# sxyu/avatar

Measured on AMD Instinct MI355X. Metric: Gauss-Newton iterations/sec (30k-pt cloud, 10 shape + 24-joint pose), higher is better.
Workload: dtype f64

## Files before the change

### avatar_amd/api.py

```python
from __future__ import annotations

import ctypes as C
import math
import os

import numpy as np

from . import capi
from .capi import AvtError, ModelArrays, Options, Profile, Stats, bptr, check, dptr, iptr


def rot_to_quat(R):
    m = np.asarray(R, np.float64).reshape(-1, 3, 3)
    N = m.shape[0]
    q = np.empty((N, 4))
    tr = m[:, 0, 0] + m[:, 1, 1] + m[:, 2, 2]
    pos = tr > 0
    with np.errstate(invalid="ignore", divide="ignore"):
        t = np.sqrt(np.where(pos, tr, 0.0) + 1.0)
        ti = 0.5 / t
        qa = np.stack([(m[:, 2, 1] - m[:, 1, 2]) * ti, (m[:, 0, 2] - m[:, 2, 0]) * ti, (m[:, 1, 0] - m[:, 0, 1]) * ti, 0.5 * t], 1)
        i = np.where(m[:, 1, 1] > m[:, 0, 0], 1, 0)
        ar = np.arange(N)
        i = np.where(m[:, 2, 2] > m[ar, i, i], 2, i)
# ... 437 lines not shown

    def normal_equations(self, frame=0):
        P = self.model.arrays.P
        H = np.empty((P, P)); g = np.empty(P); cost = C.c_double()
        check(self._lib.avt_get_normal_equations(self.h, C.c_int(frame), dptr(H), dptr(g), C.byref(cost)))
        return H, g, cost.value

    def cost_trace(self, frame=0, n=11):
        buf = np.zeros(64)
        check(self._lib.avt_debug_trace(self.h, C.c_int(frame), dptr(buf)))
        return buf[:n].copy()

    def mfma_count(self, frame=0):
        a, b, c = C.c_longlong(), C.c_longlong(), C.c_longlong()
        check(self._lib.avt_debug_mfma_count(self.h, C.c_int(frame), C.byref(a), C.byref(b), C.byref(c)))
        return {k: (None if v.value < 0 else int(v.value)) for k, v in (("eval_rows", a), ("moments", b), ("solve", c))}

    def nn_sums(self, frame=0):
        V = self.model.numPoints()
        cnt = np.empty(V, np.int32); fsum = np.empty((3, V), np.int64); centre = np.empty(3)
        check(self._lib.avt_debug_nn_sums(self.h, C.c_int(frame), iptr(cnt), fsum.ctypes.data_as(C.POINTER(C.c_longlong)), dptr(centre)))
        return cnt, fsum, centre

    DATA_TERM_ROWS, DATA_TERM_MOMENTS, DATA_TERM_AUTO = 0, 1, 2

    def tuning(self):
        t = capi.Tuning()
        check(self._lib.avt_ctx_get_tuning(self.h, C.byref(t)))
        return t

    def set_tuning(self, **kw):
        t = self.tuning()
        for k, v in kw.items():
            if k not in dict(t._fields_):
                raise KeyError(k)
            setattr(t, k, int(v))
        check(self._lib.avt_ctx_set_tuning(self.h, C.byref(t)))
        return self

    def set_data_term(self, form):
        check(self._lib.avt_set_data_term(self.h, C.c_int(int(form))))

    def data_term(self):
        return int(self._lib.avt_get_data_term(self.h))

    def launch_shape(self):
# ... 175 lines not shown
```

### avatar_amd/capi.py

```python
from __future__ import annotations

import ctypes as C
import os

import numpy as np
import scipy.sparse as sp

_HERE = os.path.dirname(os.path.abspath(__file__))
LIB_PATH = os.environ.get("AVT_LIB", os.path.join(_HERE, "csrc", "libavatar_hip.so"))

c_double_p = C.POINTER(C.c_double)
c_int_p = C.POINTER(C.c_int)
c_ubyte_p = C.POINTER(C.c_ubyte)

AVT_K_NAMES = ["lbs", "visibility", "bucket", "nn", "aggregate", "prepare", "eval", "reduce", "solve", "decide", "moments"]
AVT_K_COUNT = len(AVT_K_NAMES)


class ModelDesc(C.Structure):
    _fields_ = [
        ("num_points", C.c_int), ("num_joints", C.c_int), ("num_shape_keys", C.c_int), ("num_faces", C.c_int),
        ("base_cloud", c_double_p), ("key_clouds", c_double_p), ("parent", c_int_p), ("mesh", c_int_p),
        ("weights_colptr", c_int_p), ("weights_row", c_int_p), ("weights_val", c_double_p),
        ("jreg_colptr", c_int_p), ("jreg_row", c_int_p), ("jreg_val", c_double_p),
# ... 185 lines not shown
    "avt_state_upload_frames": [_vp, C.c_int, c_int_p, c_double_p, c_double_p, c_double_p],
    "avt_state_reset": [_vp],
    "avt_state_download": [_vp, c_double_p, c_double_p, c_double_p, C.POINTER(Stats)],
    "avt_get_correspondences": [_vp, C.c_int, c_int_p],
    "avt_get_cloud": [_vp, C.c_int, c_double_p],
    "avt_get_posed": [_vp, C.c_int, c_double_p, c_double_p, c_double_p],
    "avt_get_normal_equations": [_vp, C.c_int, c_double_p, c_double_p, c_double_p],
    "avt_ctx_get_tuning": [_vp, C.POINTER(Tuning)],
    "avt_ctx_set_tuning": [_vp, C.POINTER(Tuning)],
    "avt_set_data_term": [_vp, C.c_int],
    "avt_get_data_term": [_vp],
    "avt_set_occlusion_render": [_vp, C.c_int, C.c_int, C.c_float, C.c_float, C.c_float, C.c_float],
    "avt_get_visibility": [_vp, C.c_int, c_ubyte_p],
    "avt_set_corr_gate": [_vp, C.c_int, c_double_p],
    "avt_get_corr_gate": [_vp, c_double_p],
    "avt_get_gated": [_vp, C.c_int, c_int_p],
    "avt_set_corr_trim": [_vp, C.c_int, c_double_p, c_double_p, c_double_p, C.c_int],
    "avt_get_corr_trim": [_vp, c_double_p, c_double_p, c_double_p, c_int_p],
    "avt_get_trimmed": [_vp, C.c_int, c_int_p, c_int_p],
    "avt_get_trim_thresholds": [_vp, C.c_int, c_double_p],
    "avt_debug_trace": [_vp, C.c_int, c_double_p],
    "avt_debug_mfma_count": [_vp, C.c_int, C.POINTER(C.c_longlong), C.POINTER(C.c_longlong), C.POINTER(C.c_longlong)],
    "avt_debug_nn_sums": [_vp, C.c_int, c_int_p, C.POINTER(C.c_longlong), c_double_p],
    "avt_launch_shape": [_vp, c_int_p, c_int_p, c_int_p],
    "avt_profile_begin": [_vp],
    "avt_profile_select": [_vp, C.c_uint],
    "avt_profile_end": [_vp, C.POINTER(Profile)],
    "avt_shard_owner": [C.c_int, C.c_int],
    "avt_shard_local_count": [C.c_int, C.c_int, C.c_int],
    "avt_shard_local_index": [C.c_int, C.c_int],
    "avt_shard_global_frame": [C.c_int, C.c_int, C.c_int],
    "avt_model_pack_size": [C.POINTER(ModelDesc), C.POINTER(C.c_size_t)],
    "avt_model_pack": [C.POINTER(ModelDesc), _vp, C.c_size_t],
    "avt_model_unpack": [_vp, C.c_size_t, C.POINTER(_vp)],
    "avt_shard_unique_id": [C.c_char_p],
    "avt_shard_create": [C.c_int, C.c_int, C.c_int, C.c_char_p, C.POINTER(_vp)],
    "avt_shard_create_loopback": [C.c_int, C.c_int, C.c_int, C.c_char_p, C.POINTER(_vp)],
    "avt_shard_create_shm": [C.c_int, C.c_int, C.c_int, C.c_char_p, C.POINTER(_vp)],
    "avt_shard_destroy": [_vp],
    "avt_shard_rank": [_vp],
    "avt_shard_world": [_vp],
    "avt_shard_backend": [_vp],
    "avt_shard_broadcast_model": [_vp, C.c_int, C.POINTER(ModelDesc), C.POINTER(_vp)],
    "avt_shard_scatter_frames": [_vp, _vp, C.c_int, C.c_int, c_double_p, c_int_p, c_int_p, c_double_p, c_double_p, c_double_p],
    "avt_shard_gather_enqueue": [_vp, _vp, C.c_int],
    "avt_shard_gather_wait": [_vp],
# ... 39 lines not shown
```

### avatar_amd/csrc/avt_capi.cpp

```cpp
#include <algorithm>
#include <cmath>
#include <cstdio>
#include <cstdlib>
#include <cstring>
#include <limits>

#include <memory>
#include <mutex>

#include "avt_internal.h"

static std::mutex g_graph_mutex;

int avt_solve_set_attributes();
int avt_eval_set_attributes();
int avt_render_enqueue(avt_ctx* c, int nframes, const int* d_vertex_part, unsigned long long* d_zkey, unsigned char* d_label, int* d_block,
                       double fx, double fy, double cx, double cy, int width, int height);
int avt_paint_enqueue(avt_ctx* c, int nframes, const int* d_vertex_part, unsigned long long* d_dkey, unsigned long long* d_mkey, float* d_fkey,
                      int* d_frank, unsigned char* d_fedge, float* d_depth, unsigned char* d_label, int* d_block, double fx, double fy, double cx,
                      double cy, int width, int height);
void avt_eval_report_occupancy(const AvtDims& d);

namespace {

template <class T>
int dev_alloc(avt_ctx* c, T** p, size_t n) {
    DevBuf<char> b;
    if (b.reserve(std::max<size_t>(n, 1) * sizeof(T))) return 1;
    *p = (T*)b.p;
    c->owned.push_back(std::move(b));
    return 0;
}
template <class T>
int dev_upload(avt_ctx* c, T** p, const std::vector<T>& v) {
    if (dev_alloc(c, p, v.size())) return 1;
    if (!v.empty()) {
        AVT_HIP(hipMemcpyAsync(*p, v.data(), v.size() * sizeof(T), hipMemcpyHostToDevice, c->stream));
        AVT_HIP(hipStreamSynchronize(c->stream));
    }
    return 0;
}

int choose_groups(int nframes, const avt_tuning& tun) {
    int n = nframes >= 44 ? 2 : 1;
    if (tun.groups > 0) n = tun.groups;
    return std::max(1, std::min(std::min(n, AVT_MAX_GROUPS), nframes));
}

int choose_G(int nframes, int ngroups, const avt_tuning& tun);
int plan_groups(avt_ctx* c, int nf) {
    int ngroups = choose_groups(nf, c->tun);
    if ((nf == 2 || nf == 3) && c->tun.groups <= 0) {
        const int g_keep = c->fb.G;
        c->fb.G = choose_G(1, 1, c->tun);
        if (avt_solve_rides(c, 1)) ngroups = nf;
        c->fb.G = g_keep;
    }
    return ngroups;
}

int choose_G(int nframes, int ngroups, const avt_tuning& tun) {
    const int target = nframes >= 128 ? 1536 : (ngroups >= 2 ? (nframes <= 40 ? 512 : 640) : 768);
    const int gcap = std::max(2, std::min(AVT_G_MAX, tun.gcap));
    int g = std::max(2, std::min(gcap, target / std::max(1, nframes)));
    if (nframes >= 7) g = std::min(g, 63);
    if (tun.g > 0) return std::max(1, std::min(g, tun.g));
    return g;
}

extern "C" char** environ;
avt_tuning tuning_from_environment() {
    avt_tuning t;
    std::memset(&t, 0, sizeof t);
    t.use_graph = 1; t.groups = 0; t.g = 0; t.gcap = 128; t.vis_frame_min = 32; t.ride = 1; t.ride_strips = 0; t.ride_sizing_groups = 0;
    t.asm_parts = 1; t.spec_cost = 1; t.xcd_frames = 1; t.literal_dims = 1; t.nspec = AVT_MAX_SPEC; t.nn_force_part = 0; t.nn_force_vis = 0; t.nn_slab = 1; t.mom_min_frames = 8; t.debug = 0; t.ride_timeout_us = 2000000;
    struct Knob { const char* name; int* field; };
    const Knob knobs[] = {{"AVT_USE_GRAPH", &t.use_graph}, {"AVT_GROUPS", &t.groups}, {"AVT_G", &t.g}, {"AVT_GCAP", &t.gcap}, {"AVT_VIS_FRAME_MIN", &t.vis_frame_min},
                          {"AVT_RIDE", &t.ride}, {"AVT_RIDE_STRIPS", &t.ride_strips}, {"AVT_RIDE_SIZING_GROUPS", &t.ride_sizing_groups}, {"AVT_NSPEC", &t.nspec},
                          {"AVT_NN_FORCE_PART", &t.nn_force_part}, {"AVT_NN_FORCE_VIS", &t.nn_force_vis}, {"AVT_NN_SLAB", &t.nn_slab}, {"AVT_MOM_MIN_FRAMES", &t.mom_min_frames}, {"AVT_ASM_PARTS", &t.asm_parts}, {"AVT_LBS_FRAMES", &t.lbs_frames}, {"AVT_SPEC_COST", &t.spec_cost}, {"AVT_XCD_FRAMES", &t.xcd_frames}, {"AVT_LITERAL_DIMS", &t.literal_dims}, {"AVT_DEBUG", &t.debug}};
    const char* others[] = {"AVT_LIB", "AVT_RCCL_LIB", "AVT_SHARD_LOOPBACK_TIMEOUT_S", "AVT_BENCH_SHARE_GPU0", "AVT_TIMING"};
    for (char** e = environ; e && *e; ++e) {
        if (std::strncmp(*e, "AVT_", 4) != 0) continue;
        const char* eq = std::strchr(*e, '=');
        if (!eq) continue;
        const std::string name(*e, eq - *e);
        const char* val = eq + 1;
        bool known = false;
        for (const Knob& k : knobs) if (name == k.name) { *k.field = atoi(val); known = true; }
        if (name == "AVT_RIDE_TIMEOUT_US") { t.ride_timeout_us = std::max(0ll, atoll(val)); known = true; }
        if (name == "AVT_NO_GRAPH") { t.use_graph = 0; known = true; }
        if (name == "AVT_ONE_GROUP") { t.groups = 1; known = true; }
        if (name == "AVT_NO_RIDE") { t.ride = 0; known = true; }
        if (name == "AVT_NN_NO_SLAB") { t.nn_slab = 0; known = true; }
        if (name == "AVT_RIDE_SIZING") { t.ride_sizing_groups = std::strcmp(val, "groups") == 0; known = true; }
        for (const char* o : others) if (name == o) known = true;
        if (!known) fprintf(stderr, "libavatar_hip: environment variable %s is not a knob of this library (include/avt.h, avt_tuning) - ignored\n", name.c_str());
    }
    return t;
}

int validate_tuning(const avt_tuning& t) {
    if (t.groups < 0 || t.groups > AVT_MAX_GROUPS || t.g < 0 || t.gcap < 2 || t.vis_frame_min < 0 || t.nspec < 0 || t.nspec > AVT_MAX_SPEC ||
        (t.ride_strips != 0 && t.ride_strips != 4 && t.ride_strips != 8) || t.mom_min_frames < 1 || t.ride_timeout_us < 0 || (t.lbs_frames != 0 && t.lbs_frames != 1 && t.lbs_frames != 2 && t.lbs_frames != 4) || t.spec_cost < 0 || t.spec_cost > 1 || t.xcd_frames < 0 || t.xcd_frames > 1 || t.literal_dims < 0 || t.literal_dims > 1 || t.nn_force_vis < 0 || t.nn_force_vis > 1) {
        avt_set_error("avt_tuning: a field is out of range (include/avt.h)");
        return 1;
    }
    return 0;
}

hipEvent_t next_event(avt_ctx* c) {
    if (c->event_pool_used == c->event_pool.size()) {
// ... 406 lines not shown
    c->results_fresh = false;
    AVT_HIP(hipMemsetAsync(c->fb.fault, 0, (size_t)c->fb.max_frames * sizeof(unsigned), c->stream));
    AVT_HIP(hipStreamSynchronize(c->stream));
    return 0;
}

extern "C" {

static int ctx_create_impl(int device, const avt_model* m, int num_parts, const int* part_map, int max_points, int max_frames, avt_ctx** out) {
    if (!m || !part_map || !out) { avt_set_error("avt_ctx_create: null argument"); return 1; }
    if (num_parts <= 0 || num_parts > AVT_MAX_PARTS) { avt_set_error("avt_ctx_create: num_parts out of range (1..64)"); return 1; }
    if (max_points <= 0 || max_frames <= 0) { avt_set_error("avt_ctx_create: max_points/max_frames must be positive"); return 1; }
    int ndev = 0;
    if (hipGetDeviceCount(&ndev) != hipSuccess || ndev <= 0) {
        avt_set_error("avt_ctx_create: no HIP device available (this library has no CPU fallback)");
        return 2;
    }
    if (device < 0 || device >= ndev) { avt_set_error("avt_ctx_create: device index out of range"); return 1; }
    AVT_HIP(hipSetDevice(device));
    avt_ctx* c = new avt_ctx();
    *out = c;
    c->device = device;
    c->model = m;
    c->tun = tuning_from_environment();
    if (validate_tuning(c->tun)) return 1;
    { hipDeviceProp_t pr; c->num_cus = hipGetDeviceProperties(&pr, device) == hipSuccess ? pr.multiProcessorCount : 0; }
    AVT_HIP(hipStreamCreateWithFlags(&c->stream, hipStreamNonBlocking));
    AVT_HIP(hipEventCreateWithFlags(&c->ev_fork, hipEventDisableTiming));
    for (int i = 0; i < AVT_MAX_GROUPS - 1; ++i) {
        AVT_HIP(hipStreamCreateWithFlags(&c->side[i], hipStreamNonBlocking));
        AVT_HIP(hipEventCreateWithFlags(&c->ev_join[i], hipEventDisableTiming));
    }
    c->cur_stream = c->stream;
    if (avt_solve_set_attributes() || avt_eval_set_attributes() || avt_lbs_set_attributes() || avt_moments_set_attributes()) { avt_set_error("avt_ctx_create: hipFuncSetAttribute failed"); return 1; }
    DeviceModel& dm = c->dm;
    dm.d = m->d;
    if (!dm.d.mom_ok) c->mom_reason = "K + 1 <= 16 and 3 + 3J + K <= 87 required";
    else if (avt_moments_lds_need(dm.d) > avt_moments_lds_cap()) {
        dm.d.mom_ok = 0;
        c->mom_reason = "its assembly needs " + std::to_string(avt_moments_lds_need(dm.d)) + " bytes of LDS per workgroup, " + std::to_string(avt_moments_lds_cap()) + " available";
    }
    c->vis_frame_min = avt_visibility_frame_lds(m->d) <= 150 * 1024 ? c->tun.vis_frame_min : 0;
    dm.d.num_parts = num_parts;
    const int V = dm.d.V, J = dm.d.J;
    c->part_map.assign(part_map, part_map + J);
    std::vector<int> pov(V), pstart(num_parts + 1, 0), pverts(V), ppos(V);
    for (int v = 0; v < V; ++v) {
        const int q = part_map[m->main_joint[v]];
        if (q < 0 || q >= num_parts) { avt_set_error("avt_ctx_create: part_map entry out of [0,num_parts)"); return 1; }
        pov[v] = q;
        pstart[q + 1]++;
    }
    for (int q = 0; q < num_parts; ++q) pstart[q + 1] += pstart[q];
    {
        std::vector<int> fill(pstart.begin(), pstart.end() - 1);
        for (int v = 0; v < V; ++v) { const int pos = fill[pov[v]]++; pverts[pos] = v; ppos[v] = pos; }
    }
    if (dev_upload(c, &dm.vrec, m->vrec) || dev_upload(c, &dm.shape_planes, m->shape_planes) || dev_upload(c, &dm.lbs_w, m->lbs_w) || dev_upload(c, &dm.lbs_j, m->lbs_j) ||
        dev_upload(c, &dm.asg_w, m->asg_w) || dev_upload(c, &dm.asg_j, m->asg_j) || dev_upload(c, &dm.anc_n, m->anc_n) ||
        dev_upload(c, &dm.anc, m->anc) || dev_upload(c, &dm.mesh, m->mesh_soa) || dev_upload(c, &dm.parent, m->parent) || dev_upload(c, &dm.jlevel, m->jlevel) || dev_upload(c, &dm.fk_items, m->fk_items) || dev_upload(c, &dm.tile_col, m->tile_col) || dev_upload(c, &dm.deal_col, m->deal_col) || dev_upload(c, &dm.tile_param, m->tile_param) ||
        dev_upload(c, &dm.joint_col, m->joint_col) || dev_upload(c, &dm.vorder, m->vorder) || dev_upload(c, &dm.vmask, m->vmask) || dev_upload(c, &dm.fk_level_off, m->fk_level_off) || dev_upload(c, &dm.fk_titems, m->fk_titems) ||
        dev_upload(c, &dm.jsr_base, m->jsr_base) || dev_upload(c, &dm.jsr, m->jsr) || dev_upload(c, &dm.S, m->S) ||
        dev_upload(c, &dm.Sp, m->Sp) || dev_upload(c, &dm.prior_mean, m->prior_mean) || dev_upload(c, &dm.prior_prec, m->prior_prec) ||
        dev_upload(c, &dm.prior_clog, m->prior_clog) || dev_upload(c, &dm.part_of_vertex, pov) ||
        dev_upload(c, &dm.part_start, pstart) || dev_upload(c, &dm.part_vertices, pverts) || dev_upload(c, &dm.part_pos, ppos) ||
        dev_upload(c, &dm.mom_pair, m->mom_pair) || dev_upload(c, &dm.mom_lstart, m->mom_lstart) || dev_upload(c, &dm.mom_lv, m->mom_lv) || dev_upload(c, &dm.mom_lw, m->mom_lw) ||
        dev_upload(c, &dm.mom_psi, m->mom_psi) || dev_upload(c, &dm.mom_opk_start, m->mom_opk_start) || dev_upload(c, &dm.mom_opk, m->mom_opk) ||
        dev_upload(c, &dm.mom_sub_start, m->mom_sub_start) || dev_upload(c, &dm.mom_sub, m->mom_sub) || dev_upload(c, &dm.mom_m1_start, m->mom_m1_start) ||
        dev_upload(c, &dm.mom_m1, m->mom_m1) || dev_upload(c, &dm.mom_s2_start, m->mom_s2_start) || dev_upload(c, &dm.mom_s2, m->mom_s2) || dev_upload(c, &dm.mom_s2_jj, m->mom_s2_jj) || dev_upload(c, &dm.mom_z2_jj, m->mom_z2_jj) || dev_upload(c, &dm.mom_tab16, m->mom_tab16))
        return 1;
    FrameBuffers& fb = c->fb;
    fb.max_frames = max_frames;
    fb.max_points = max_points;
    fb.G = choose_G(max_frames, 1, c->tun);
    fb.const_blocks = (max_points + 255) / 256;
    fb.bucket_tiles = (max_points + 2047) / 2048;
    const size_t FN = (size_t)max_frames * max_points, FV = (size_t)max_frames * V;
    const AvtDims& d = dm.d;
    size_t part_cap = 0;
    avt_tuning widest = c->tun;
    widest.gcap = AVT_G_MAX; widest.g = 0;
    for (int nf = 1; nf <= max_frames; ++nf)
        for (int k = 1; k <= std::min(AVT_MAX_GROUPS, nf); ++k) part_cap = std::max(part_cap, (size_t)nf * std::max(choose_G((nf + k - 1) / k, 1, widest), choose_G((nf + k - 1) / k, 2, widest)));
    char* cntsum = nullptr;
    char* state_block = nullptr;
    if (dev_alloc(c, &fb.data_raw, FN * 3) || dev_alloc(c, &fb.labels_raw, FN) || dev_alloc(c, &fb.dx, FN) || dev_alloc(c, &fb.dy, FN) ||
        dev_alloc(c, &fb.dz, FN) || dev_alloc(c, &fb.dorig, FN) || dev_alloc(c, &fb.part_off, (size_t)max_frames * (num_parts + 1)) || dev_alloc(c, &fb.part_cnt, (size_t)max_frames * 2 * (AVT_MAX_PARTS + 1)) || dev_alloc(c, &fb.tile_hist, (size_t)max_frames * ((max_points + 2047) / 2048) * (AVT_MAX_PARTS + 1)) ||
        dev_alloc(c, &fb.corr, FN) || dev_alloc(c, &fb.corr_sorted, FN) || dev_alloc(c, &fb.cloud, FV * 3) || dev_alloc(c, &fb.pcx, FV) ||
        dev_alloc(c, &fb.pcy, FV) || dev_alloc(c, &fb.pcz, FV) || dev_alloc(c, &fb.visible, FV) || dev_alloc(c, &fb.vcx, FV) || dev_alloc(c, &fb.vcy, FV) ||
        dev_alloc(c, &fb.vcz, FV) || dev_alloc(c, &fb.vcid, FV) || dev_alloc(c, &fb.vcount, (size_t)max_frames * num_parts) || dev_alloc(c, &fb.vis_sorted, FV) || dev_alloc(c, &fb.ride_ctr, (size_t)max_frames) || dev_alloc(c, &fb.fault, (size_t)max_frames) || dev_alloc(c, &fb.spec, (size_t)max_frames) || dev_alloc(c, &fb.snap, (size_t)max_frames) || dev_alloc(c, &fb.x_spec, (size_t)max_frames * AVT_MAX_SPEC * d.xsize) || dev_alloc(c, &fb.prep_spec, (size_t)max_frames * AVT_MAX_SPEC * d.prep_size) ||
        dev_alloc(c, &cntsum, FV * (sizeof(int) + 3 * sizeof(long long)) + 64) || dev_alloc(c, &fb.matched, FV) ||
        dev_alloc(c, &fb.const_part, (size_t)max_frames * fb.const_blocks) ||
        dev_alloc(c, &state_block, 2 * ((size_t)max_frames * 2 * d.xsize * sizeof(double) + (size_t)max_frames * sizeof(AvtFrameCtl))) ||
        dev_alloc(c, &fb.prep, (size_t)max_frames * 2 * d.prep_size) ||
        dev_alloc(c, &fb.rec, (size_t)max_frames * d.nb_max * 4 * d.rec_quad) || dev_alloc(c, &fb.partial, part_cap * d.NPAIR * 256) || dev_alloc(c, &fb.wmask, part_cap) || dev_alloc(c, &fb.bmask, (size_t)max_frames * d.nb_max) || dev_alloc(c, &fb.erange, (size_t)max_frames * AVT_ERANGE) || dev_alloc(c, &fb.Hraw, (size_t)max_frames * 2 * d.HS * d.HS) ||
        dev_alloc(c, &fb.prior, (size_t)max_frames * 2 * AVT_MAX_COMPS * AVT_PRIOR_STRIDE) ||
        dev_alloc(c, &fb.jointpos, (size_t)max_frames * 3 * J) || dev_alloc(c, &fb.jointtrans, (size_t)max_frames * 12 * J) ||
        dev_alloc(c, &fb.trace, (size_t)max_frames * 64) || dev_alloc(c, &fb.results, (size_t)max_frames * result_stride(d)))
        return 1;
    {
        const size_t bx = (size_t)max_frames * 2 * d.xsize * sizeof(double), bc = (size_t)max_frames * sizeof(AvtFrameCtl);
        fb.x = (double*)state_block; fb.ctl = (AvtFrameCtl*)(state_block + bx);
        fb.x_start = (double*)(state_block + bx + bc); fb.ctl_start = (AvtFrameCtl*)(state_block + 2 * bx + bc);
    }
    if (d.mom_ok) {
        if (dev_alloc(c, &fb.mom_T, (size_t)max_frames * avt_moments_T_doubles(d)) || dev_alloc(c, &fb.mom_D, (size_t)max_frames * J * d.mom_npsi * 3) ||
            dev_alloc(c, &fb.mom_E, (size_t)max_frames * 2) || dev_alloc(c, &fb.mom_rec, (size_t)max_frames * avt_moments_frame_scratch(d)))
            return 1;
        AVT_HIP(hipMemsetAsync(fb.mom_D, 0, (size_t)max_frames * J * d.mom_npsi * 3 * sizeof(double), c->stream));
    }
    {
        AvtRunParams* pr = nullptr;
        if (dev_alloc(c, &pr, 1)) return 1;
        fb.params = pr;
    }
    {
        double* g2 = nullptr;
        if (dev_alloc(c, &g2, (size_t)num_parts) || dev_alloc(c, &fb.gated, (size_t)max_frames)) return 1;
        fb.gate2 = g2;
        c->gate_host.assign((size_t)num_parts, std::numeric_limits<double>::infinity());
        c->gate2_host = c->gate_host;
        AVT_HIP(hipMemcpyAsync(g2, c->gate2_host.data(), (size_t)num_parts * sizeof(double), hipMemcpyHostToDevice, c->stream));
        AVT_HIP(hipMemsetAsync(fb.gated, 0, (size_t)max_frames * sizeof(int), c->stream));
    }
    fb.spec_frames = std::min(max_frames, AVT_SPEC_FRAMES);
    if (dev_alloc(c, &fb.partial_spec, (size_t)fb.spec_frames * AVT_MAX_SPEC * AVT_G_MAX * 256) || dev_alloc(c, &fb.wmask_spec, (size_t)fb.spec_frames * AVT_MAX_SPEC * AVT_G_MAX) ||
        dev_alloc(c, &fb.prior_spec, (size_t)fb.spec_frames * AVT_MAX_SPEC * AVT_MAX_COMPS * AVT_PRIOR_STRIDE))
        return 1;
    fb.fsum = (long long*)cntsum;
    fb.cnt = (int*)(cntsum + FV * 3 * sizeof(long long));
    AVT_HIP(hipMemsetAsync(fb.trace, 0, (size_t)max_frames * 64 * sizeof(double), c->stream));
    AVT_HIP(hipMemsetAsync(fb.ctl, 0, (size_t)max_frames * sizeof(AvtFrameCtl), c->stream));
    AVT_HIP(hipMemsetAsync(fb.ride_ctr, 0, (size_t)max_frames * sizeof(unsigned), c->stream));
    AVT_HIP(hipMemsetAsync(fb.fault, 0, (size_t)max_frames * sizeof(unsigned), c->stream));
    fb.ride_timeout = c->tun.ride_timeout_us * 100;
    fb.xcd_frames = c->tun.xcd_frames;
    AVT_HIP(hipMemsetAsync(fb.spec, 0, (size_t)max_frames * sizeof(AvtSpecCtl), c->stream));
    AVT_HIP(hipMemsetAsync(fb.part_cnt, 0, (size_t)max_frames * 2 * (AVT_MAX_PARTS + 1) * sizeof(int), c->stream));
    AVT_HIP(hipStreamSynchronize(c->stream));
    if (c->tun.debug) avt_eval_report_occupancy(dm.d);
    return 0;
}


int avt_ctx_create(int device, const avt_model* m, int num_parts, const int* part_map, int max_points, int max_frames, avt_ctx** out) {
    if (out) *out = nullptr;
    const int rc = avt_guard("avt_ctx_create", [&]() -> int { return ctx_create_impl(device, m, num_parts, part_map, max_points, max_frames, out); });
    if (rc != 0 && out && *out) {
        const std::string keep = avt_last_error();
        avt_ctx_destroy(*out);
        *out = nullptr;
// ... 641 lines not shown

int avt_get_trim_thresholds(avt_ctx* c, int frame, double* T) {
    return avt_guard("avt_get_trim_thresholds", [&]() -> int {
        if (!c || !T) { avt_set_error("avt_get_trim_thresholds: null argument"); return 1; }
        if (trim_search_ran(c, "avt_get_trim_thresholds", frame)) return 1;
        const int np = c->dm.d.num_parts;
        if (!c->trim_last) { std::fill(T, T + np, std::numeric_limits<double>::infinity()); return 0; }
        AVT_HIP(hipSetDevice(c->device));
        AVT_HIP(hipMemcpyAsync(T, c->trim_thr.p + (size_t)frame * np, (size_t)np * sizeof(double), hipMemcpyDeviceToHost, c->stream));
        AVT_HIP(hipStreamSynchronize(c->stream));
        return 0;
    });
}

int avt_get_visibility(avt_ctx* c, int frame, unsigned char* visible) {
    if (!c || !visible || frame < 0 || frame >= c->nframes) { avt_set_error("avt_get_visibility: bad argument"); return 1; }
    if (!c->frames_valid || c->ran_icp_iters <= 0) { avt_set_error("avt_get_visibility: no optimize call with an ICP iteration has run on the resident frames"); return 1; }
    AVT_HIP(hipSetDevice(c->device));
    AVT_HIP(hipMemcpyAsync(visible, c->fb.visible + (size_t)frame * c->dm.d.V, (size_t)c->dm.d.V, hipMemcpyDeviceToHost, c->stream));
    AVT_HIP(hipStreamSynchronize(c->stream));
    return 0;
}

int avt_debug_trace(avt_ctx* c, int frame, double* out64) {
    if (!c || !out64 || frame < 0 || frame >= c->fb.max_frames) { avt_set_error("avt_debug_trace: bad argument"); return 1; }
    AVT_HIP(hipSetDevice(c->device));
    AVT_HIP(hipStreamSynchronize(c->stream));
    AVT_HIP(hipMemcpyAsync(out64, c->fb.trace + (size_t)frame * 64, 64 * sizeof(double), hipMemcpyDeviceToHost, c->stream));
    AVT_HIP(hipStreamSynchronize(c->stream));
    return 0;
}

int avt_launch_shape(avt_ctx* c, int* groups, int* frames_per_group, int* eval_workgroups_per_frame) {
    if (!c || c->nframes <= 0) { avt_set_error("avt_launch_shape: no frames resident"); return 1; }
    const int use_moments_keep = c->fb.use_moments;
    c->fb.use_moments = choose_moments(c, c->nframes);
    const int ng = plan_groups(c, c->nframes), nfg = (c->nframes + ng - 1) / ng;
    c->fb.use_moments = use_moments_keep;
    if (groups) *groups = ng;
    if (frames_per_group) *frames_per_group = nfg;
    if (eval_workgroups_per_frame) *eval_workgroups_per_frame = choose_G(nfg, ng, c->tun);
    return 0;
}

int avt_profile_begin(avt_ctx* c) {
    if (!c) { avt_set_error("avt_profile_begin: null context"); return 1; }
// ... 31 lines not shown
```

### avatar_amd/csrc/avt_internal.h

```cpp
#pragma once
#include <hip/hip_runtime.h>

#include <map>
#include <string>
#include <vector>

#include "../../include/avt.h"
#include "../../include/avt_shard.h"
#include "avt_host.h"

#define AVT_ANC_MAX 16
#define AVT_TILE 16
#define AVT_EVAL_PTS 16
#define AVT_EVAL_ROWS (3 * AVT_EVAL_PTS)
#define AVT_EVAL_RS 49
#define AVT_EVAL_TILE(ncols) ((((ncols) * AVT_EVAL_RS) + 1) & ~1)
#define AVT_ERANGE 66
#define AVT_MAX_TILES 12
#define AVT_MAX_P 179
#define AVT_MAX_COMPS 16
#define AVT_G_MAX 128
#define AVT_MAX_GROUPS 4
#define AVT_PRIOR_STRIDE (2 + 3 * AVT_MAX_JOINTS)
#define AVT_FIX_SCALE 1099511627776.0
// ... 289 lines not shown

struct AvtSubState {
    DevBuf<int> block;
    DevBuf<int> in;
    DevBuf<double> out;
    std::vector<int> h_in;
    std::vector<double> h_out;
    std::vector<int> counts;
    hipEvent_t ev_labels = nullptr;
    bool pending = false;
    int prev_nframes = -1;
};

struct avt_ctx {
    int device = 0;
    hipStream_t stream = nullptr;
    hipStream_t side[AVT_MAX_GROUPS - 1] = {};
    hipEvent_t ev_fork = nullptr, ev_join[AVT_MAX_GROUPS - 1] = {};
    hipStream_t cur_stream = nullptr;
    const avt_model* model = nullptr;
    DeviceModel dm = {};
    FrameBuffers fb = {};
    std::vector<DevBuf<char>> owned;
    std::vector<int> part_map;
    int nframes = 0;
    std::vector<int> frame_N, frame_off;
    bool profiling = false;
    unsigned prof_mask = 0xffffffffu;
    std::vector<std::pair<int, std::pair<hipEvent_t, hipEvent_t>>> prof_events;
    std::vector<hipEvent_t> event_pool;
    size_t event_pool_used = 0;
    int ran_icp_iters = 0, ran_max_iters = 0;
    int launch_maxN = 0;
    int num_cus = 0;
    bool lbs_cleared = false;
    bool nn_from_cloud = false;
    bool scatter_in_compact = false;
    int vis_frame_min = 0;
    struct GraphEntry { std::string key; hipGraphExec_t exec; unsigned long long last_used; };
    std::vector<GraphEntry> graphs;
    unsigned long long graph_clock = 0;
    AvtRunParams params_host = {};
    std::vector<double> gate_host, gate2_host;
    std::vector<double> trim_rho, trim_kappa, trim_floor, trim_set_host;
    int trim_min_matches = 1;
    bool trim_on = false, trim_last = false;
// ... 68 lines not shown
```

### include/avt.h

```cpp
#ifndef AVT_H_
#define AVT_H_

#ifdef __cplusplus
extern "C" {
#endif

#define AVT_STATUS_NO_DEVICE 2
#define AVT_STATUS_DEVICE_FAULT 3

#define AVT_MAX_JOINTS 64
#define AVT_MAX_SHAPE 16
#define AVT_MAX_ASSIGN 4
#define AVT_MAX_PARTS 64

typedef struct avt_model avt_model;
typedef struct avt_ctx avt_ctx;

typedef struct avt_model_desc {
    int num_points;
    int num_joints;
    int num_shape_keys;
    int num_faces;
    const double* base_cloud;
    const double* key_clouds;
// ... 112 lines not shown
                            double cx, double cy, int width, int height, int* points_per_frame);
enum { AVT_RENDER_ZBUFFER = 0, AVT_RENDER_PAINTER = 1 };
int avt_synth_render_frames_mode(avt_ctx* c, int nframes, const double* w, const double* p, const double* R, double fx, double fy,
                                 double cx, double cy, int width, int height, int mode, int* points_per_frame);
int avt_synth_render_images(avt_ctx* c, int frame, float* depth_HxW, unsigned char* part_mask_HxW);
int avt_frames_download(avt_ctx* c, int frame, double* data_3xN, int* labels);

int avt_get_correspondences(avt_ctx* c, int frame, int* model_idx_out );
int avt_get_cloud(avt_ctx* c, int frame, double* cloud_3xV);
int avt_get_visibility(avt_ctx* c, int frame, unsigned char* visible_V);
int avt_get_posed(avt_ctx* c, int frame, double* cloud_3xV, double* joint_pos_3xJ, double* joint_trans_12xJ);
int avt_get_normal_equations(avt_ctx* c, int frame, double* H , double* g , double* cost);

enum { AVT_DATA_TERM_ROWS = 0, AVT_DATA_TERM_MOMENTS = 1, AVT_DATA_TERM_AUTO = 2 };
int avt_set_data_term(avt_ctx* c, int form);
int avt_get_data_term(avt_ctx* c);

int avt_debug_trace(avt_ctx* c, int frame, double* out64);

int avt_debug_mfma_count(avt_ctx* c, int frame, long long* eval_rows, long long* moments, long long* solve);

int avt_debug_nn_sums(avt_ctx* c, int frame, int* cnt, long long* fsum, double* centre);

typedef struct avt_tuning {
    int use_graph;
    int groups;
    int g;
    int gcap;
    int vis_frame_min;
    int ride;
    int ride_strips;
    int ride_sizing_groups;
    int nspec;
    int nn_force_part;
    int nn_slab;
    int mom_min_frames;
    int debug;
    int asm_parts;
    long long ride_timeout_us;
    int lbs_frames;
    int spec_cost;
    int xcd_frames;
    int literal_dims;
    int nn_force_vis;
} avt_tuning;
int avt_ctx_get_tuning(avt_ctx* c, avt_tuning* out);
// ... 13 lines not shown
```

Before: 26140.

## Pack device buffers into one page-aligned arena grouped by access hotness

Replaces the many separate device allocations at context creation with a single 2MB-aligned arena. Buffers are ordered by rank: hot small per-frame and model buffers come first, followed by small cold and then bulk buffers. Model uploads are staged into one contiguous host copy. The aim is to cut TLB misses and scattered small-buffer accesses in the per-iteration kernels, and to reduce setup cost. In exchange the arena is zero-filled on creation, and buffers now sit next to each other, so an out-of-bounds write in one kernel could silently corrupt a neighbouring buffer.

```diff
diff --git a/avatar_amd/api.py b/avatar_amd/api.py
--- a/avatar_amd/api.py
+++ b/avatar_amd/api.py
@@ -483,6 +483,18 @@
         check(self._lib.avt_debug_nn_sums(self.h, C.c_int(frame), iptr(cnt), fsum.ctypes.data_as(C.POINTER(C.c_longlong)), dptr(centre)))
         return cnt, fsum, centre
 
+    def arena(self):
+        base, nbytes, count = C.c_ulonglong(), C.c_ulonglong(), C.c_int()
+        check(self._lib.avt_debug_arena(self.h, C.byref(base), C.byref(nbytes), C.byref(count)))
+        entries = []
+        for i in range(count.value):
+            off, n = C.c_ulonglong(), C.c_ulonglong()
+            name = C.create_string_buffer(64)
+            check(self._lib.avt_debug_arena_entry(self.h, C.c_int(i), C.byref(off), C.byref(n)))
+            check(self._lib.avt_debug_arena_name(self.h, C.c_int(i), name, C.c_int(64)))
+            entries.append((name.value.decode(), off.value, n.value))
+        return dict(base=base.value, bytes=nbytes.value, entries=entries)
+
     DATA_TERM_ROWS, DATA_TERM_MOMENTS, DATA_TERM_AUTO = 0, 1, 2
 
     def tuning(self):
diff --git a/avatar_amd/capi.py b/avatar_amd/capi.py
--- a/avatar_amd/capi.py
+++ b/avatar_amd/capi.py
@@ -231,6 +231,10 @@
     "avt_debug_trace": [_vp, C.c_int, c_double_p],
     "avt_debug_mfma_count": [_vp, C.c_int, C.POINTER(C.c_longlong), C.POINTER(C.c_longlong), C.POINTER(C.c_longlong)],
     "avt_debug_nn_sums": [_vp, C.c_int, c_int_p, C.POINTER(C.c_longlong), c_double_p],
+    "avt_debug_arena": [_vp, C.POINTER(C.c_ulonglong), C.POINTER(C.c_ulonglong), c_int_p],
+    "avt_debug_arena_entry": [_vp, C.c_int, C.POINTER(C.c_ulonglong), C.POINTER(C.c_ulonglong)],
+    "avt_debug_arena_name": [_vp, C.c_int, C.c_char_p, C.c_int],
+    "avt_arena_plan": [C.c_int, C.POINTER(C.c_size_t), c_int_p, C.POINTER(C.c_size_t), C.POINTER(C.c_size_t)],
     "avt_launch_shape": [_vp, c_int_p, c_int_p, c_int_p],
     "avt_profile_begin": [_vp],
     "avt_profile_select": [_vp, C.c_uint],
diff --git a/avatar_amd/csrc/avt_arena.cpp b/avatar_amd/csrc/avt_arena.cpp
--- /dev/null
+++ b/avatar_amd/csrc/avt_arena.cpp
@@ -0,0 +1,35 @@
+#include "avt_arena.h"
+
+#include <vector>
+
+namespace {
+
+bool round_up(size_t a, size_t align, size_t* out) {
+    size_t s;
+    if (__builtin_add_overflow(a, align - 1, &s)) return false;
+    *out = s & ~(align - 1);
+    return true;
+}
+
+}
+
+extern "C" int avt_arena_plan(int n, const size_t* bytes, const int* rank, size_t* offsets, size_t* total) {
+    if (n < 0 || (n > 0 && (!bytes || !offsets)) || !total) return 1;
+    for (int i = 0; i < n; ++i)
+        if (rank && (rank[i] < 0 || rank[i] >= AVT_RANK_COUNT)) return 1;
+    std::vector<size_t> off((size_t)n);
+    size_t cur = 0;
+    for (int r = 0; r < AVT_RANK_COUNT; ++r)
+        for (int i = 0; i < n; ++i) {
+            if ((rank ? rank[i] : 0) != r) continue;
+            const size_t align = bytes[i] >= AVT_ARENA_ALIGN_BIG ? AVT_ARENA_ALIGN_BIG : AVT_ARENA_ALIGN;
+            if (!round_up(cur, align, &cur)) return 1;
+            off[(size_t)i] = cur;
+            if (__builtin_add_overflow(cur, bytes[i] ? bytes[i] : (size_t)1, &cur)) return 1;
+        }
+    size_t end;
+    if (__builtin_add_overflow(cur, AVT_ARENA_TAIL, &end) || !round_up(end, AVT_ARENA_PAGE, &end)) return 1;
+    for (int i = 0; i < n; ++i) offsets[i] = off[(size_t)i];
+    *total = end;
+    return 0;
+}
diff --git a/avatar_amd/csrc/avt_arena.h b/avatar_amd/csrc/avt_arena.h
--- /dev/null
+++ b/avatar_amd/csrc/avt_arena.h
@@ -0,0 +1,20 @@
+#pragma once
+#include <cstddef>
+
+constexpr size_t AVT_ARENA_ALIGN = 256;
+constexpr size_t AVT_ARENA_ALIGN_BIG = 64 * 1024;
+constexpr size_t AVT_ARENA_BULK = 256 * 1024;
+constexpr size_t AVT_ARENA_PAGE = 2 * 1024 * 1024;
+constexpr size_t AVT_ARENA_TAIL = 4096;
+
+enum AvtArenaRank { AVT_RANK_HOT_FRAME = 0, AVT_RANK_HOT_MODEL = 1, AVT_RANK_SMALL_MODEL = 2, AVT_RANK_BULK_MODEL = 3, AVT_RANK_SMALL_FRAME = 4, AVT_RANK_BULK_FRAME = 5, AVT_RANK_COUNT = 6 };
+
+inline int avt_arena_rank(size_t bytes, bool model, bool hot) {
+    if (bytes >= AVT_ARENA_BULK) return model ? AVT_RANK_BULK_MODEL : AVT_RANK_BULK_FRAME;
+    if (hot) return model ? AVT_RANK_HOT_MODEL : AVT_RANK_HOT_FRAME;
+    return model ? AVT_RANK_SMALL_MODEL : AVT_RANK_SMALL_FRAME;
+}
+
+extern "C" {
+int avt_arena_plan(int n, const size_t* bytes, const int* rank, size_t* offsets, size_t* total);
+}
diff --git a/avatar_amd/csrc/avt_capi.cpp b/avatar_amd/csrc/avt_capi.cpp
--- a/avatar_amd/csrc/avt_capi.cpp
+++ b/avatar_amd/csrc/avt_capi.cpp
@@ -8,6 +8,7 @@
 #include <memory>
 #include <mutex>
 
+#include "avt_arena.h"
 #include "avt_internal.h"
 
 static std::mutex g_graph_mutex;
@@ -23,19 +24,63 @@
 
 namespace {
 
-template <class T>
-int dev_alloc(avt_ctx* c, T** p, size_t n) {
-    DevBuf<char> b;
-    if (b.reserve(std::max<size_t>(n, 1) * sizeof(T))) return 1;
-    *p = (T*)b.p;
-    c->owned.push_back(std::move(b));
-    return 0;
-}
-template <class T>
-int dev_upload(avt_ctx* c, T** p, const std::vector<T>& v) {
-    if (dev_alloc(c, p, v.size())) return 1;
-    if (!v.empty()) {
-        AVT_HIP(hipMemcpyAsync(*p, v.data(), v.size() * sizeof(T), hipMemcpyHostToDevice, c->stream));
+struct ArenaBuilder {
+    struct Req { const char* name; void** slot; size_t bytes; int rank; const void* src; size_t src_bytes; };
+    std::vector<Req> reqs;
+    bool model = true;
+    template <class T>
+    void add(const char* name, T** p, size_t n, bool hot = false, const void* src = nullptr) {
+        const size_t bytes = std::max<size_t>(n, 1) * sizeof(T);
+        *p = nullptr;
+        reqs.push_back({name, (void**)p, bytes, avt_arena_rank(bytes, model, hot), src, src ? n * sizeof(T) : 0});
+    }
+    template <class T>
+    void upload(const char* name, T** p, const std::vector<T>& v, bool hot = false) { add(name, p, v.size(), hot, v.empty() ? nullptr : v.data()); }
+};
+
+int arena_commit(avt_ctx* c, const ArenaBuilder& ab) {
+    const int n = (int)ab.reqs.size();
+    if (!c->use_arena) {
+        for (const ArenaBuilder::Req& r : ab.reqs) {
+            DevBuf<char> b;
+            if (b.reserve(r.bytes)) return 1;
+            *r.slot = b.p;
+            c->owned.push_back(std::move(b));
+            if (r.src_bytes) {
+                AVT_HIP(hipMemcpyAsync(*r.slot, r.src, r.src_bytes, hipMemcpyHostToDevice, c->stream));
+                AVT_HIP(hipStreamSynchronize(c->stream));
+            }
+        }
+        return 0;
+    }
+    std::vector<size_t> bytes((size_t)n), off((size_t)n);
+    std::vector<int> rank((size_t)n);
+    for (int i = 0; i < n; ++i) { bytes[i] = ab.reqs[i].bytes; rank[i] = ab.reqs[i].rank; }
+    size_t total = 0;
+    if (avt_arena_plan(n, bytes.data(), rank.data(), off.data(), &total)) { avt_set_error("avt_ctx_create: the sizes of the device buffers do not fit size_t"); return 1; }
+    DevBuf<char> block;
+    if (block.reserve(total)) return 1;
+    char* base = block.p;
+    if ((uintptr_t)base % AVT_ARENA_PAGE) {
+        if (block.reserve(total + AVT_ARENA_PAGE)) return 1;
+        base = block.p + (AVT_ARENA_PAGE - (uintptr_t)block.p % AVT_ARENA_PAGE) % AVT_ARENA_PAGE;
+    }
+    c->owned.push_back(std::move(block));
+    c->arena_base = base;
+    c->arena_bytes = total;
+    AVT_HIP(hipMemsetAsync(base, 0, total, c->stream));
+    size_t lo = total, hi = 0;
+    for (int i = 0; i < n; ++i) {
+        const ArenaBuilder::Req& r = ab.reqs[i];
+        *r.slot = base + off[i];
+        c->arena_entries.push_back({r.name, off[i], r.bytes});
+        if (r.src_bytes) { lo = std::min(lo, off[i]); hi = std::max(hi, off[i] + r.src_bytes); }
+    }
+    if (hi > lo) {
+        std::vector<char> stage(hi - lo, 0);
+        for (int i = 0; i < n; ++i)
+            if (ab.reqs[i].src_bytes) std::memcpy(stage.data() + (off[i] - lo), ab.reqs[i].src, ab.reqs[i].src_bytes);
+        AVT_HIP(hipMemcpyAsync(base + lo, stage.data(), hi - lo, hipMemcpyHostToDevice, c->stream));
         AVT_HIP(hipStreamSynchronize(c->stream));
     }
     return 0;
@@ -69,7 +114,7 @@
 }
 
 extern "C" char** environ;
-avt_tuning tuning_from_environment() {
+avt_tuning tuning_from_environment(int* use_arena) {
     avt_tuning t;
     std::memset(&t, 0, sizeof t);
     t.use_graph = 1; t.groups = 0; t.g = 0; t.gcap = 128; t.vis_frame_min = 32; t.ride = 1; t.ride_strips = 0; t.ride_sizing_groups = 0;
@@ -78,6 +123,7 @@
     const Knob knobs[] = {{"AVT_USE_GRAPH", &t.use_graph}, {"AVT_GROUPS", &t.groups}, {"AVT_G", &t.g}, {"AVT_GCAP", &t.gcap}, {"AVT_VIS_FRAME_MIN", &t.vis_frame_min},
                           {"AVT_RIDE", &t.ride}, {"AVT_RIDE_STRIPS", &t.ride_strips}, {"AVT_RIDE_SIZING_GROUPS", &t.ride_sizing_groups}, {"AVT_NSPEC", &t.nspec},
                           {"AVT_NN_FORCE_PART", &t.nn_force_part}, {"AVT_NN_FORCE_VIS", &t.nn_force_vis}, {"AVT_NN_SLAB", &t.nn_slab}, {"AVT_MOM_MIN_FRAMES", &t.mom_min_frames}, {"AVT_ASM_PARTS", &t.asm_parts}, {"AVT_LBS_FRAMES", &t.lbs_frames}, {"AVT_SPEC_COST", &t.spec_cost}, {"AVT_XCD_FRAMES", &t.xcd_frames}, {"AVT_LITERAL_DIMS", &t.literal_dims}, {"AVT_DEBUG", &t.debug}};
+    *use_arena = 1;
     const char* others[] = {"AVT_LIB", "AVT_RCCL_LIB", "AVT_SHARD_LOOPBACK_TIMEOUT_S", "AVT_BENCH_SHARE_GPU0", "AVT_TIMING"};
     for (char** e = environ; e && *e; ++e) {
         if (std::strncmp(*e, "AVT_", 4) != 0) continue;
@@ -87,6 +133,7 @@
         const char* val = eq + 1;
         bool known = false;
         for (const Knob& k : knobs) if (name == k.name) { *k.field = atoi(val); known = true; }
+        if (name == "AVT_ARENA") { *use_arena = atoi(val) != 0; known = true; }
         if (name == "AVT_RIDE_TIMEOUT_US") { t.ride_timeout_us = std::max(0ll, atoll(val)); known = true; }
         if (name == "AVT_NO_GRAPH") { t.use_graph = 0; known = true; }
         if (name == "AVT_ONE_GROUP") { t.groups = 1; known = true; }
@@ -539,7 +586,7 @@
     *out = c;
     c->device = device;
     c->model = m;
-    c->tun = tuning_from_environment();
+    c->tun = tuning_from_environment(&c->use_arena);
     if (validate_tuning(c->tun)) return 1;
     { hipDeviceProp_t pr; c->num_cus = hipGetDeviceProperties(&pr, device) == hipSuccess ? pr.multiProcessorCount : 0; }
     AVT_HIP(hipStreamCreateWithFlags(&c->stream, hipStreamNonBlocking));
@@ -573,19 +620,24 @@
         std::vector<int> fill(pstart.begin(), pstart.end() - 1);
         for (int v = 0; v < V; ++v) { const int pos = fill[pov[v]]++; pverts[pos] = v; ppos[v] = pos; }
     }
-    if (dev_upload(c, &dm.vrec, m->vrec) || dev_upload(c, &dm.shape_planes, m->shape_planes) || dev_upload(c, &dm.lbs_w, m->lbs_w) || dev_upload(c, &dm.lbs_j, m->lbs_j) ||
-        dev_upload(c, &dm.asg_w, m->asg_w) || dev_upload(c, &dm.asg_j, m->asg_j) || dev_upload(c, &dm.anc_n, m->anc_n) ||
-        dev_upload(c, &dm.anc, m->anc) || dev_upload(c, &dm.mesh, m->mesh_soa) || dev_upload(c, &dm.parent, m->parent) || dev_upload(c, &dm.jlevel, m->jlevel) || dev_upload(c, &dm.fk_items, m->fk_items) || dev_upload(c, &dm.tile_col, m->tile_col) || dev_upload(c, &dm.deal_col, m->deal_col) || dev_upload(c, &dm.tile_param, m->tile_param) ||
-        dev_upload(c, &dm.joint_col, m->joint_col) || dev_upload(c, &dm.vorder, m->vorder) || dev_upload(c, &dm.vmask, m->vmask) || dev_upload(c, &dm.fk_level_off, m->fk_level_off) || dev_upload(c, &dm.fk_titems, m->fk_titems) ||
-        dev_upload(c, &dm.jsr_base, m->jsr_base) || dev_upload(c, &dm.jsr, m->jsr) || dev_upload(c, &dm.S, m->S) ||
-        dev_upload(c, &dm.Sp, m->Sp) || dev_upload(c, &dm.prior_mean, m->prior_mean) || dev_upload(c, &dm.prior_prec, m->prior_prec) ||
-        dev_upload(c, &dm.prior_clog, m->prior_clog) || dev_upload(c, &dm.part_of_vertex, pov) ||
-        dev_upload(c, &dm.part_start, pstart) || dev_upload(c, &dm.part_vertices, pverts) || dev_upload(c, &dm.part_pos, ppos) ||
-        dev_upload(c, &dm.mom_pair, m->mom_pair) || dev_upload(c, &dm.mom_lstart, m->mom_lstart) || dev_upload(c, &dm.mom_lv, m->mom_lv) || dev_upload(c, &dm.mom_lw, m->mom_lw) ||
-        dev_upload(c, &dm.mom_psi, m->mom_psi) || dev_upload(c, &dm.mom_opk_start, m->mom_opk_start) || dev_upload(c, &dm.mom_opk, m->mom_opk) ||
-        dev_upload(c, &dm.mom_sub_start, m->mom_sub_start) || dev_upload(c, &dm.mom_sub, m->mom_sub) || dev_upload(c, &dm.mom_m1_start, m->mom_m1_start) ||
-        dev_upload(c, &dm.mom_m1, m->mom_m1) || dev_upload(c, &dm.mom_s2_start, m->mom_s2_start) || dev_upload(c, &dm.mom_s2, m->mom_s2) || dev_upload(c, &dm.mom_s2_jj, m->mom_s2_jj) || dev_upload(c, &dm.mom_z2_jj, m->mom_z2_jj) || dev_upload(c, &dm.mom_tab16, m->mom_tab16))
-        return 1;
+    ArenaBuilder ab;
+#define AVT_UP(field, vec, ...) ab.upload(#field, &field, vec, ##__VA_ARGS__)
+#define AVT_AL(field, n, ...) ab.add(#field, &field, n, ##__VA_ARGS__)
+    const bool HOT = true;
+    AVT_UP(dm.vrec, m->vrec); AVT_UP(dm.shape_planes, m->shape_planes); AVT_UP(dm.lbs_w, m->lbs_w); AVT_UP(dm.lbs_j, m->lbs_j);
+    AVT_UP(dm.asg_w, m->asg_w); AVT_UP(dm.asg_j, m->asg_j); AVT_UP(dm.anc_n, m->anc_n);
+    AVT_UP(dm.anc, m->anc); AVT_UP(dm.mesh, m->mesh_soa); AVT_UP(dm.parent, m->parent, HOT); AVT_UP(dm.jlevel, m->jlevel, HOT); AVT_UP(dm.fk_items, m->fk_items, HOT);
+    AVT_UP(dm.tile_col, m->tile_col, HOT); AVT_UP(dm.deal_col, m->deal_col, HOT); AVT_UP(dm.tile_param, m->tile_param, HOT);
+    AVT_UP(dm.joint_col, m->joint_col, HOT); AVT_UP(dm.vorder, m->vorder); AVT_UP(dm.vmask, m->vmask); AVT_UP(dm.fk_level_off, m->fk_level_off, HOT); AVT_UP(dm.fk_titems, m->fk_titems, HOT);
+    AVT_UP(dm.jsr_base, m->jsr_base, HOT); AVT_UP(dm.jsr, m->jsr, HOT); AVT_UP(dm.S, m->S, HOT);
+    AVT_UP(dm.Sp, m->Sp, HOT); AVT_UP(dm.prior_mean, m->prior_mean, HOT); AVT_UP(dm.prior_prec, m->prior_prec, HOT);
+    AVT_UP(dm.prior_clog, m->prior_clog, HOT); AVT_UP(dm.part_of_vertex, pov);
+    AVT_UP(dm.part_start, pstart); AVT_UP(dm.part_vertices, pverts); AVT_UP(dm.part_pos, ppos);
+    AVT_UP(dm.mom_pair, m->mom_pair); AVT_UP(dm.mom_lstart, m->mom_lstart); AVT_UP(dm.mom_lv, m->mom_lv); AVT_UP(dm.mom_lw, m->mom_lw);
+    AVT_UP(dm.mom_psi, m->mom_psi); AVT_UP(dm.mom_opk_start, m->mom_opk_start); AVT_UP(dm.mom_opk, m->mom_opk);
+    AVT_UP(dm.mom_sub_start, m->mom_sub_start); AVT_UP(dm.mom_sub, m->mom_sub); AVT_UP(dm.mom_m1_start, m->mom_m1_start);
+    AVT_UP(dm.mom_m1, m->mom_m1); AVT_UP(dm.mom_s2_start, m->mom_s2_start); AVT_UP(dm.mom_s2, m->mom_s2); AVT_UP(dm.mom_s2_jj, m->mom_s2_jj); AVT_UP(dm.mom_z2_jj, m->mom_z2_jj); AVT_UP(dm.mom_tab16, m->mom_tab16);
+    ab.model = false;
     FrameBuffers& fb = c->fb;
     fb.max_frames = max_frames;
     fb.max_points = max_points;
@@ -601,49 +653,47 @@
         for (int k = 1; k <= std::min(AVT_MAX_GROUPS, nf); ++k) part_cap = std::max(part_cap, (size_t)nf * std::max(choose_G((nf + k - 1) / k, 1, widest), choose_G((nf + k - 1) / k, 2, widest)));
     char* cntsum = nullptr;
     char* state_block = nullptr;
-    if (dev_alloc(c, &fb.data_raw, FN * 3) || dev_alloc(c, &fb.labels_raw, FN) || dev_alloc(c, &fb.dx, FN) || dev_alloc(c, &fb.dy, FN) ||
-        dev_alloc(c, &fb.dz, FN) || dev_alloc(c, &fb.dorig, FN) || dev_alloc(c, &fb.part_off, (size_t)max_frames * (num_parts + 1)) || dev_alloc(c, &fb.part_cnt, (size_t)max_frames * 2 * (AVT_MAX_PARTS + 1)) || dev_alloc(c, &fb.tile_hist, (size_t)max_frames * ((max_points + 2047) / 2048) * (AVT_MAX_PARTS + 1)) ||
-        dev_alloc(c, &fb.corr, FN) || dev_alloc(c, &fb.corr_sorted, FN) || dev_alloc(c, &fb.cloud, FV * 3) || dev_alloc(c, &fb.pcx, FV) ||
-        dev_alloc(c, &fb.pcy, FV) || dev_alloc(c, &fb.pcz, FV) || dev_alloc(c, &fb.visible, FV) || dev_alloc(c, &fb.vcx, FV) || dev_alloc(c, &fb.vcy, FV) ||
-        dev_alloc(c, &fb.vcz, FV) || dev_alloc(c, &fb.vcid, FV) || dev_alloc(c, &fb.vcount, (size_t)max_frames * num_parts) || dev_alloc(c, &fb.vis_sorted, FV) || dev_alloc(c, &fb.ride_ctr, (size_t)max_frames) || dev_alloc(c, &fb.fault, (size_t)max_frames) || dev_alloc(c, &fb.spec, (size_t)max_frames) || dev_alloc(c, &fb.snap, (size_t)max_frames) || dev_alloc(c, &fb.x_spec, (size_t)max_frames * AVT_MAX_SPEC * d.xsize) || dev_alloc(c, &fb.prep_spec, (size_t)max_frames * AVT_MAX_SPEC * d.prep_size) ||
-        dev_alloc(c, &cntsum, FV * (sizeof(int) + 3 * sizeof(long long)) + 64) || dev_alloc(c, &fb.matched, FV) ||
-        dev_alloc(c, &fb.const_part, (size_t)max_frames * fb.const_blocks) ||
-        dev_alloc(c, &state_block, 2 * ((size_t)max_frames * 2 * d.xsize * sizeof(double) + (size_t)max_frames * sizeof(AvtFrameCtl))) ||
-        dev_alloc(c, &fb.prep, (size_t)max_frames * 2 * d.prep_size) ||
-        dev_alloc(c, &fb.rec, (size_t)max_frames * d.nb_max * 4 * d.rec_quad) || dev_alloc(c, &fb.partial, part_cap * d.NPAIR * 256) || dev_alloc(c, &fb.wmask, part_cap) || dev_alloc(c, &fb.bmask, (size_t)max_frames * d.nb_max) || dev_alloc(c, &fb.erange, (size_t)max_frames * AVT_ERANGE) || dev_alloc(c, &fb.Hraw, (size_t)max_frames * 2 * d.HS * d.HS) ||
-        dev_alloc(c, &fb.prior, (size_t)max_frames * 2 * AVT_MAX_COMPS * AVT_PRIOR_STRIDE) ||
-        dev_alloc(c, &fb.jointpos, (size_t)max_frames * 3 * J) || dev_alloc(c, &fb.jointtrans, (size_t)max_frames * 12 * J) ||
-        dev_alloc(c, &fb.trace, (size_t)max_frames * 64) || dev_alloc(c, &fb.results, (size_t)max_frames * result_stride(d)))
-        return 1;
+    AVT_AL(fb.data_raw, FN * 3); AVT_AL(fb.labels_raw, FN); AVT_AL(fb.dx, FN); AVT_AL(fb.dy, FN);
+    AVT_AL(fb.dz, FN); AVT_AL(fb.dorig, FN); AVT_AL(fb.part_off, (size_t)max_frames * (num_parts + 1), HOT); AVT_AL(fb.part_cnt, (size_t)max_frames * 2 * (AVT_MAX_PARTS + 1), HOT); AVT_AL(fb.tile_hist, (size_t)max_frames * ((max_points + 2047) / 2048) * (AVT_MAX_PARTS + 1));
+    AVT_AL(fb.corr, FN); AVT_AL(fb.corr_sorted, FN); AVT_AL(fb.cloud, FV * 3); AVT_AL(fb.pcx, FV);
+    AVT_AL(fb.pcy, FV); AVT_AL(fb.pcz, FV); AVT_AL(fb.visible, FV); AVT_AL(fb.vcx, FV); AVT_AL(fb.vcy, FV);
+    AVT_AL(fb.vcz, FV); AVT_AL(fb.vcid, FV); AVT_AL(fb.vcount, (size_t)max_frames * num_parts, HOT); AVT_AL(fb.vis_sorted, FV); AVT_AL(fb.ride_ctr, (size_t)max_frames, HOT); AVT_AL(fb.fault, (size_t)max_frames, HOT); AVT_AL(fb.spec, (size_t)max_frames, HOT); AVT_AL(fb.snap, (size_t)max_frames, HOT); AVT_AL(fb.x_spec, (size_t)max_frames * AVT_MAX_SPEC * d.xsize, HOT); AVT_AL(fb.prep_spec, (size_t)max_frames * AVT_MAX_SPEC * d.prep_size, HOT);
+    AVT_AL(cntsum, FV * (sizeof(int) + 3 * sizeof(long long)) + 64); AVT_AL(fb.matched, FV);
+    AVT_AL(fb.const_part, (size_t)max_frames * fb.const_blocks, HOT);
+    AVT_AL(state_block, 2 * ((size_t)max_frames * 2 * d.xsize * sizeof(double) + (size_t)max_frames * sizeof(AvtFrameCtl)), HOT);
+    AVT_AL(fb.prep, (size_t)max_frames * 2 * d.prep_size, HOT);
+    AVT_AL(fb.rec, (size_t)max_frames * d.nb_max * 4 * d.rec_quad); AVT_AL(fb.partial, part_cap * d.NPAIR * 256); AVT_AL(fb.wmask, part_cap, HOT); AVT_AL(fb.bmask, (size_t)max_frames * d.nb_max, HOT); AVT_AL(fb.erange, (size_t)max_frames * AVT_ERANGE, HOT); AVT_AL(fb.Hraw, (size_t)max_frames * 2 * d.HS * d.HS, HOT);
+    AVT_AL(fb.prior, (size_t)max_frames * 2 * AVT_MAX_COMPS * AVT_PRIOR_STRIDE, HOT);
+    AVT_AL(fb.jointpos, (size_t)max_frames * 3 * J, HOT); AVT_AL(fb.jointtrans, (size_t)max_frames * 12 * J, HOT);
+    AVT_AL(fb.trace, (size_t)max_frames * 64, HOT); AVT_AL(fb.results, (size_t)max_frames * result_stride(d), HOT);
+    if (d.mom_ok) {
+        AVT_AL(fb.mom_T, (size_t)max_frames * avt_moments_T_doubles(d)); AVT_AL(fb.mom_D, (size_t)max_frames * J * d.mom_npsi * 3);
+        AVT_AL(fb.mom_E, (size_t)max_frames * 2, HOT); AVT_AL(fb.mom_rec, (size_t)max_frames * avt_moments_frame_scratch(d));
+    }
+    AvtRunParams* params = nullptr;
+    AVT_AL(params, 1, HOT);
+    double* gate2 = nullptr;
+    AVT_AL(gate2, (size_t)num_parts, HOT); AVT_AL(fb.gated, (size_t)max_frames, HOT);
+    fb.spec_frames = std::min(max_frames, AVT_SPEC_FRAMES);
+    AVT_AL(fb.partial_spec, (size_t)fb.spec_frames * AVT_MAX_SPEC * AVT_G_MAX * 256); AVT_AL(fb.wmask_spec, (size_t)fb.spec_frames * AVT_MAX_SPEC * AVT_G_MAX, HOT);
+    AVT_AL(fb.prior_spec, (size_t)fb.spec_frames * AVT_MAX_SPEC * AVT_MAX_COMPS * AVT_PRIOR_STRIDE, HOT);
+#undef AVT_UP
+#undef AVT_AL
+    if (arena_commit(c, ab)) return 1;
     {
         const size_t bx = (size_t)max_frames * 2 * d.xsize * sizeof(double), bc = (size_t)max_frames * sizeof(AvtFrameCtl);
         fb.x = (double*)state_block; fb.ctl = (AvtFrameCtl*)(state_block + bx);
         fb.x_start = (double*)(state_block + bx + bc); fb.ctl_start = (AvtFrameCtl*)(state_block + 2 * bx + bc);
     }
-    if (d.mom_ok) {
-        if (dev_alloc(c, &fb.mom_T, (size_t)max_frames * avt_moments_T_doubles(d)) || dev_alloc(c, &fb.mom_D, (size_t)max_frames * J * d.mom_npsi * 3) ||
-            dev_alloc(c, &fb.mom_E, (size_t)max_frames * 2) || dev_alloc(c, &fb.mom_rec, (size_t)max_frames * avt_moments_frame_scratch(d)))
-            return 1;
-        AVT_HIP(hipMemsetAsync(fb.mom_D, 0, (size_t)max_frames * J * d.mom_npsi * 3 * sizeof(double), c->stream));
-    }
+    if (d.mom_ok) AVT_HIP(hipMemsetAsync(fb.mom_D, 0, (size_t)max_frames * J * d.mom_npsi * 3 * sizeof(double), c->stream));
+    fb.params = params;
     {
-        AvtRunParams* pr = nullptr;
-        if (dev_alloc(c, &pr, 1)) return 1;
-        fb.params = pr;
-    }
-    {
-        double* g2 = nullptr;
-        if (dev_alloc(c, &g2, (size_t)num_parts) || dev_alloc(c, &fb.gated, (size_t)max_frames)) return 1;
-        fb.gate2 = g2;
+        fb.gate2 = gate2;
         c->gate_host.assign((size_t)num_parts, std::numeric_limits<double>::infinity());
         c->gate2_host = c->gate_host;
-        AVT_HIP(hipMemcpyAsync(g2, c->gate2_host.data(), (size_t)num_parts * sizeof(double), hipMemcpyHostToDevice, c->stream));
+        AVT_HIP(hipMemcpyAsync(gate2, c->gate2_host.data(), (size_t)num_parts * sizeof(double), hipMemcpyHostToDevice, c->stream));
         AVT_HIP(hipMemsetAsync(fb.gated, 0, (size_t)max_frames * sizeof(int), c->stream));
     }
-    fb.spec_frames = std::min(max_frames, AVT_SPEC_FRAMES);
-    if (dev_alloc(c, &fb.partial_spec, (size_t)fb.spec_frames * AVT_MAX_SPEC * AVT_G_MAX * 256) || dev_alloc(c, &fb.wmask_spec, (size_t)fb.spec_frames * AVT_MAX_SPEC * AVT_G_MAX) ||
-        dev_alloc(c, &fb.prior_spec, (size_t)fb.spec_frames * AVT_MAX_SPEC * AVT_MAX_COMPS * AVT_PRIOR_STRIDE))
-        return 1;
     fb.fsum = (long long*)cntsum;
     fb.cnt = (int*)(cntsum + FV * 3 * sizeof(long long));
     AVT_HIP(hipMemsetAsync(fb.trace, 0, (size_t)max_frames * 64 * sizeof(double), c->stream));
@@ -1331,6 +1381,27 @@
     return 0;
 }
 
+int avt_debug_arena(avt_ctx* c, unsigned long long* base, unsigned long long* bytes, int* count) {
+    if (!c) { avt_set_error("avt_debug_arena: bad argument"); return 1; }
+    if (base) *base = (unsigned long long)(uintptr_t)c->arena_base;
+    if (bytes) *bytes = c->arena_bytes;
+    if (count) *count = (int)c->arena_entries.size();
+    return 0;
+}
+
+int avt_debug_arena_entry(avt_ctx* c, int i, unsigned long long* offset, unsigned long long* bytes) {
+    if (!c || i < 0 || i >= (int)c->arena_entries.size()) { avt_set_error("avt_debug_arena_entry: bad argument"); return 1; }
+    if (offset) *offset = c->arena_entries[(size_t)i].offset;
+    if (bytes) *bytes = c->arena_entries[(size_t)i].bytes;
+    return 0;
+}
+
+int avt_debug_arena_name(avt_ctx* c, int i, char* name, int cap) {
+    if (!c || !name || cap <= 0 || i < 0 || i >= (int)c->arena_entries.size()) { avt_set_error("avt_debug_arena_name: bad argument"); return 1; }
+    std::snprintf(name, (size_t)cap, "%s", c->arena_entries[(size_t)i].name);
+    return 0;
+}
+
 int avt_debug_trace(avt_ctx* c, int frame, double* out64) {
     if (!c || !out64 || frame < 0 || frame >= c->fb.max_frames) { avt_set_error("avt_debug_trace: bad argument"); return 1; }
     AVT_HIP(hipSetDevice(c->device));
diff --git a/avatar_amd/csrc/avt_internal.h b/avatar_amd/csrc/avt_internal.h
--- a/avatar_amd/csrc/avt_internal.h
+++ b/avatar_amd/csrc/avt_internal.h
@@ -335,6 +335,11 @@
     DeviceModel dm = {};
     FrameBuffers fb = {};
     std::vector<DevBuf<char>> owned;
+    int use_arena = 1;
+    char* arena_base = nullptr;
+    size_t arena_bytes = 0;
+    struct ArenaEntry { const char* name; size_t offset, bytes; };
+    std::vector<ArenaEntry> arena_entries;
     std::vector<int> part_map;
     int nframes = 0;
     std::vector<int> frame_N, frame_off;
diff --git a/include/avt.h b/include/avt.h
--- a/include/avt.h
+++ b/include/avt.h
@@ -1,5 +1,7 @@
 #ifndef AVT_H_
 #define AVT_H_
+
+#include <stddef.h>
 
 #ifdef __cplusplus
 extern "C" {
@@ -158,6 +160,11 @@
 
 int avt_debug_nn_sums(avt_ctx* c, int frame, int* cnt, long long* fsum, double* centre);
 
+int avt_debug_arena(avt_ctx* c, unsigned long long* base, unsigned long long* bytes, int* count);
+int avt_debug_arena_entry(avt_ctx* c, int i, unsigned long long* offset, unsigned long long* bytes);
+int avt_debug_arena_name(avt_ctx* c, int i, char* name, int cap);
+int avt_arena_plan(int n, const size_t* bytes, const int* rank, size_t* offsets, size_t* total);
+
 typedef struct avt_tuning {
     int use_graph;
     int groups;
```

New measurement: 26040. Within noise of the previous version (-0.4%).
